# TuringLang/AdvancedHMC.jl

Measured on AMD Instinct MI355X. Metric: leapfrog-steps/sec (whole node) at n_chains x D, higher is better.
Workload: dtype f64

## Files before the change

advancedhmc.jl_amd/csrc/ahmc_device.hpp:

```cpp
#pragma once

#include <hip/hip_runtime.h>
#include <stdint.h>

namespace ahmc {

enum : uint32_t { RNG_MOMENTUM = 0, RNG_TRANSITION = 1, RNG_JITTER = 2, RNG_FINDEPS = 3 };
constexpr uint32_t COUPLED_CHAIN = 0xFFFFFFFFu;

struct Philox4 {
  uint32_t v[4];
};

__device__ __forceinline__ Philox4 philox4x32_10(uint32_t c0, uint32_t c1, uint32_t c2, uint32_t c3,
                                                 uint32_t k0, uint32_t k1) {
  constexpr uint32_t M0 = 0xD2511F53u, M1 = 0xCD9E8D57u, W0 = 0x9E3779B9u, W1 = 0xBB67AE85u;
#pragma unroll
  for (int round = 0; round < 10; ++round) {
    uint32_t hi0 = __umulhi(M0, c0), lo0 = M0 * c0;
    uint32_t hi1 = __umulhi(M1, c2), lo1 = M1 * c2;
    uint32_t n0 = hi1 ^ c1 ^ k0, n2 = hi0 ^ c3 ^ k1;
    c0 = n0; c1 = lo1; c2 = n2; c3 = lo0;
    k0 += W0; k1 += W1;
  }
// ... 154 lines not shown
__device__ __forceinline__ float leaf_weight_exp(float x) { return exp(x); }

template <class T, bool UNIFORM>
__device__ __forceinline__ T alpha_from_logweight(T lw) {
  const T w = leaf_weight_exp<UNIFORM>(lw > T(0) ? T(0) : lw);
  return w >= T(1) ? T(1) : w;
}

template <int LA, int LB>
__device__ __forceinline__ double leaf_weight_exp_pair(double x, bool odd) {
  constexpr auto C = [](unsigned long long bits) { return __builtin_bit_cast(double, bits); };
  const double xc = x < -1100.0 ? -1100.0 : x;
  const double dk = __builtin_rint(xc * 92.33248261689366);
  double t = __builtin_fma(dk, -0x1.62e42fef00000p-7, xc);
  t = __builtin_fma(dk, -0x1.473de6af278edp-40, t);
  const int k = (int)dk;
  const int ka = __builtin_amdgcn_readlane(k, LA), kb = __builtin_amdgcn_readlane(k, LB);
  const double tja = C(EXP2_64_BITS[ka & 63]), tjb = C(EXP2_64_BITS[kb & 63]);
  const double tj = odd ? tjb : tja;
  double q = __builtin_fma(t, 8.3333333333333332e-03, 4.1666666666666664e-02);
  q = fma3(t, q, 1.6666666666666666e-01);
  q = fma3(t, q, 0.5);
  q = fma3(t, q, 1.0);
  q = q * t;
  return __builtin_ldexp(__builtin_fma(tj, q, tj), k >> 6);
}
template <int LA, int LB>
__device__ __forceinline__ float leaf_weight_exp_pair(float x, bool) { return exp(x); }

template <int L0>
__device__ __forceinline__ double leaf_weight_exp_quad(double x, bool odd, bool up) {
  constexpr auto C = [](unsigned long long bits) { return __builtin_bit_cast(double, bits); };
  const double xc = x < -1100.0 ? -1100.0 : x;
  const double dk = __builtin_rint(xc * 92.33248261689366);
  double t = __builtin_fma(dk, -0x1.62e42fef00000p-7, xc);
  t = __builtin_fma(dk, -0x1.473de6af278edp-40, t);
  const int k = (int)dk;
  const int k0 = __builtin_amdgcn_readlane(k, L0), k1 = __builtin_amdgcn_readlane(k, L0 + 1);
  const int k2 = __builtin_amdgcn_readlane(k, L0 + 2), k3 = __builtin_amdgcn_readlane(k, L0 + 3);
  const double tj0 = C(EXP2_64_BITS[k0 & 63]), tj1 = C(EXP2_64_BITS[k1 & 63]);
  const double tj2 = C(EXP2_64_BITS[k2 & 63]), tj3 = C(EXP2_64_BITS[k3 & 63]);
  const double tjl = odd ? tj1 : tj0, tjh = odd ? tj3 : tj2;
  const double tj = up ? tjh : tjl;
  double q = __builtin_fma(t, 8.3333333333333332e-03, 4.1666666666666664e-02);
  q = fma3(t, q, 1.6666666666666666e-01);
  q = fma3(t, q, 0.5);
  q = fma3(t, q, 1.0);
  q = q * t;
  return __builtin_ldexp(__builtin_fma(tj, q, tj), k >> 6);
}
template <int L0>
__device__ __forceinline__ float leaf_weight_exp_quad(float x, bool, bool) { return exp(x); }

template <class T> __device__ __forceinline__ T maxabs(T a, T b) { return fabs(a) > fabs(b) ? a : b; }

template <int CTRL> __device__ __forceinline__ int dpp_i32(int v) {
  return __builtin_amdgcn_mov_dpp(v, CTRL, 0xf, 0xf, true);
}
template <int CTRL> __device__ __forceinline__ float dpp_mov(float v) {
  return __int_as_float(dpp_i32<CTRL>(__float_as_int(v)));
}
template <int CTRL> __device__ __forceinline__ double dpp_mov(double v) {
  int lo = __double2loint(v), hi = __double2hiint(v);
  return __hiloint2double(dpp_i32<CTRL>(hi), dpp_i32<CTRL>(lo));
}
__device__ __forceinline__ float swz16(float v) {
  return __int_as_float(__builtin_amdgcn_ds_swizzle(__float_as_int(v), 0x401F));
}
__device__ __forceinline__ double swz16(double v) {
  int lo = __builtin_amdgcn_ds_swizzle(__double2loint(v), 0x401F);
  int hi = __builtin_amdgcn_ds_swizzle(__double2hiint(v), 0x401F);
  return __hiloint2double(hi, lo);
}
__device__ __forceinline__ float xor16_sum(float v) {
  auto p = __builtin_amdgcn_permlane16_swap(__float_as_int(v), __float_as_int(v), false, false);
  return __int_as_float(p[0]) + __int_as_float(p[1]);
}
__device__ __forceinline__ double xor16_sum(double v) {
  auto lo = __builtin_amdgcn_permlane16_swap(__double2loint(v), __double2loint(v), false, false);
  auto hi = __builtin_amdgcn_permlane16_swap(__double2hiint(v), __double2hiint(v), false, false);
  return __hiloint2double(hi[0], lo[0]) + __hiloint2double(hi[1], lo[1]);
}
__device__ __forceinline__ float xor32_sum(float v) {
  auto p = __builtin_amdgcn_permlane32_swap(__float_as_int(v), __float_as_int(v), false, false);
  return __int_as_float(p[0]) + __int_as_float(p[1]);
}
__device__ __forceinline__ double xor32_sum(double v) {
  auto lo = __builtin_amdgcn_permlane32_swap(__double2loint(v), __double2loint(v), false, false);
  auto hi = __builtin_amdgcn_permlane32_swap(__double2hiint(v), __double2hiint(v), false, false);
  return __hiloint2double(hi[0], lo[0]) + __hiloint2double(hi[1], lo[1]);
}

#ifndef AHMC_MFMA_REDUCE
#define AHMC_MFMA_REDUCE 0
#endif
template <class T> struct MfmaRed;
template <> struct MfmaRed<double> {
  typedef double acc_t __attribute__((ext_vector_type(4)));
  static __device__ __forceinline__ acc_t mma(double a, double b, acc_t c) { return __builtin_amdgcn_mfma_f64_16x16x4f64(a, b, c, 0, 0, 0); }
  static constexpr unsigned SEL = 8u;
  static constexpr int RA = 0, RB = 2;
};
template <> struct MfmaRed<float> {
  typedef float acc_t __attribute__((ext_vector_type(4)));
  static __device__ __forceinline__ acc_t mma(float a, float b, acc_t c) { return __builtin_amdgcn_mfma_f32_16x16x4f32(a, b, c, 0, 0, 0); }
  static constexpr unsigned SEL = 1u;
// ... 107 lines not shown

#ifndef AHMC_PAIR_RED_QUAD
#define AHMC_PAIR_RED_QUAD 1
#endif
template <class T, int Q = AHMC_PAIR_RED_QUAD>
__device__ __forceinline__ bool wave64_pair_reduce(T da, T db, T& ea, T& eb) {
  static_assert(Q >= 0 && Q <= 3, "a row has four quads");
  const bool odd = (threadIdx.x & 1u) != 0, up = (threadIdx.x & 2u) != 0;
  const T x = (odd ? db : da) + dpp_mov<0xB1>(odd ? da : db);
  const T y = (odd ? eb : ea) + dpp_mov<0xB1>(odd ? ea : eb);
  T z = (up ? y : x) + dpp_mov<0x4E>(up ? x : y);
  z += dpp_mov<0x124>(z);
  z += dpp_mov<0x128>(z);
  z = xor16_sum(z);
  z = xor32_sum(z);
  const bool le0 = (__builtin_amdgcn_ballot_w64(z <= T(0)) & 3ull) != 0ull;
  ea = dpp_mov<0x150 + 4 * Q + 2>(z);
  eb = dpp_mov<0x150 + 4 * Q + 3>(z);
  return le0;
}
template <class T>
__device__ __forceinline__ bool wave64_pair_reduce_t(T da, T db, T ea, T eb, T& z) {
  const bool odd = (threadIdx.x & 1u) != 0, up = (threadIdx.x & 2u) != 0;
  const T x = (odd ? db : da) + dpp_mov<0xB1>(odd ? da : db);
  const T y = (odd ? eb : ea) + dpp_mov<0xB1>(odd ? ea : eb);
  z = (up ? y : x) + dpp_mov<0x4E>(up ? x : y);
  z += dpp_mov<0x124>(z);
  z += dpp_mov<0x128>(z);
  z = xor16_sum(z);
  z = xor32_sum(z);
  return (__builtin_amdgcn_ballot_w64(z <= T(0)) & 3ull) != 0ull;
}

template <class T>
__device__ __forceinline__ T wave64_quad_pair(T a, T b) {
  const bool odd = (threadIdx.x & 1u) != 0;
  return (odd ? b : a) + dpp_mov<0xB1>(odd ? a : b);
}
template <class T>
__device__ __forceinline__ unsigned long long wave64_quad_reduce_t(T xab, T xcd, T xl, T yab, T ycd, T& w) {
  const bool up = (threadIdx.x & 2u) != 0, oq = (threadIdx.x & 4u) != 0, hq = (threadIdx.x & 8u) != 0;
  const T rd = (up ? xcd : xab) + dpp_mov<0x4E>(up ? xab : xcd);
  const T re = (up ? ycd : yab) + dpp_mov<0x4E>(up ? yab : ycd);
  const T rl = xl + dpp_mov<0x4E>(xl);
  const T z = (oq ? re : rd) + dpp_mov<0x124>(oq ? rd : re);
  const T zl = rl + dpp_mov<0x124>(rl);
  w = (hq ? zl : z) + dpp_mov<0x128>(hq ? z : zl);
  w = xor16_sum(w);
  w = xor32_sum(w);
  return __builtin_amdgcn_ballot_w64(w <= T(0));
}
constexpr unsigned long long QUAD_TURN_AB = 0x3ull, QUAD_TURN_CD = 0xCull, QUAD_TURN_L1 = 0x300ull;

template <int G, class T, int K>
__device__ __forceinline__ void wave_allsum(T (&v)[K]) {
  static_assert(G == 1 || G == 2 || G == 4 || G == 8 || G == 16 || G == 32 || G == 64, "bad group size");
  if constexpr (G >= 16 && K == 4) {
    wave_allsum4<G>(v[0], v[1], v[2], v[3]);
    return;
  }
  if constexpr (G >= 16 && K % 2 == 0) {
#pragma unroll
    for (int k = 0; k < K; k += 2) wave_allsum2<G>(v[k], v[k + 1]);
    return;
  }
  if constexpr (G >= 2) {
#pragma unroll
    for (int k = 0; k < K; ++k) v[k] += dpp_mov<0xB1>(v[k]);
  }
  if constexpr (G >= 4) {
#pragma unroll
    for (int k = 0; k < K; ++k) v[k] += dpp_mov<0x4E>(v[k]);
  }
  if constexpr (G >= 8) {
#pragma unroll
    for (int k = 0; k < K; ++k) v[k] += dpp_mov<0x141>(v[k]);
  }
  if constexpr (G >= 16) {
#pragma unroll
    for (int k = 0; k < K; ++k) v[k] += dpp_mov<0x140>(v[k]);
  }
  if constexpr (G >= 32) {
#pragma unroll
    for (int k = 0; k < K; ++k) {
      if constexpr ((AHMC_DS_REDUCE & 1) != 0) v[k] += ds_swz<SWZ_XOR16>(v[k]); else v[k] = xor16_sum(v[k]);
    }
  }
  if constexpr (G >= 64) {
#pragma unroll
    for (int k = 0; k < K; ++k) {
      if constexpr ((AHMC_DS_REDUCE & 1) != 0) v[k] += ds_xor32(v[k]); else v[k] = xor32_sum(v[k]);
    }
  }
}
__device__ __forceinline__ double* xwave_buf() {
  __shared__ __attribute__((aligned(16))) double buf[8 * 8];
  return buf;
}

template <int G, class T, int K>
__device__ __forceinline__ void group_allsum(T (&v)[K]) {
  if constexpr (G <= 64) {
    wave_allsum<G>(v);
  } else {
    static_assert(G == 128 || G == 256 || G == 512, "bad multi-wave group size");
    static_assert(K <= 8, "at most 8 values per reduction");
// ... 365 lines not shown
  }
  const unsigned long long m_redo = __builtin_amdgcn_ballot_w64(lw > lw_limit);
  const unsigned long long m_div = __builtin_amdgcn_ballot_w64(!(-H0 < delta_max + ne));
  o.w[0] = readlane_t<LA>(w);
  o.w[1] = readlane_t<LB>(w);
  o.sa[0] = readlane_t<LA>(sa);
  o.sa[1] = readlane_t<LB>(sa);
  o.dH[0] = readlane_t<LA>(dH);
  o.dH[1] = readlane_t<LB>(dH);
  o.redo[0] = LINW && ((m_redo >> LA) & 1ull) != 0ull;
  o.redo[1] = LINW && ((m_redo >> LB) & 1ull) != 0ull;
  o.div[0] = ((m_div >> LA) & 1ull) != 0ull;
  o.div[1] = ((m_div >> LB) & 1ull) != 0ull;
}

__device__ __forceinline__ float readlane_at(float v, int l) { return __int_as_float(__builtin_amdgcn_readlane(__float_as_int(v), l)); }
__device__ __forceinline__ double readlane_at(double v, int l) {
  return __hiloint2double(__builtin_amdgcn_readlane(__double2hiint(v), l), __builtin_amdgcn_readlane(__double2loint(v), l));
}
template <class T> struct QuadLeafStats {
  static constexpr int L0 = 4;
  T w_l, sa_l, dH_l;
  unsigned long long m_redo, m_div;
  __device__ __forceinline__ T w(int k) const { return readlane_at(w_l, L0 + k); }
  __device__ __forceinline__ T sa(int k) const { return readlane_at(sa_l, L0 + k); }
  __device__ __forceinline__ T dH(int k) const { return readlane_at(dH_l, L0 + k); }
  __device__ __forceinline__ bool redo(int k) const { return ((m_redo >> (L0 + k)) & 1ull) != 0ull; }
  __device__ __forceinline__ bool div(int k) const { return ((m_div >> (L0 + k)) & 1ull) != 0ull; }
};
template <class T, bool LINW>
__device__ __forceinline__ void quad_leaf_stats(T wz, T H0, T delta_max, T lw_limit, QuadLeafStats<T>& o) {
  constexpr int L0 = QuadLeafStats<T>::L0;
  const bool odd = (threadIdx.x & 1u) != 0, up = (threadIdx.x & 2u) != 0, oq = (threadIdx.x & 4u) != 0;
  const T from_prev = dpp_mov<0x124>(wz);
  const T ne = neg_energy_sanitized(oq ? wz : from_prev);
  const T dH = -ne - H0;
  const T lw = H0 + ne;
  T w, sa;
  if constexpr (LINW) {
    w = leaf_weight_exp_quad<L0>(lw, odd, up);
    sa = w >= T(1) ? T(1) : w;
  } else {
    const T wa = leaf_weight_exp_quad<L0>(lw > T(0) ? T(0) : lw, odd, up);
    sa = wa >= T(1) ? T(1) : wa;
    w = lw;
  }
  o.m_redo = LINW ? __builtin_amdgcn_ballot_w64(lw > lw_limit) : 0ull;
  o.m_div = __builtin_amdgcn_ballot_w64(!(-H0 < delta_max + ne));
  o.w_l = w;
  o.sa_l = sa;
  o.dH_l = dH;
}

template <class T, int G, int E, int TK, class F>
__device__ __forceinline__ void leapfrog_step_plus2(Point<T, E>& z, const T (&minv)[E], T eps, const TargetP<T>& tp, int lane, int d0,
                                                    T (&extra)[2], F&& partials, bool use_pre = false) {
  const T eh = eps / 2;
#pragma unroll
  for (int e = 0; e < E; ++e) z.r[e] = leapfrog_kick(z.r[e], eh, z.g[e]);
#pragma unroll
  for (int e = 0; e < E; ++e) z.th[e] = leapfrog_drift(z.th[e], eps, minv[e], z.r[e]);
  T red[4];
  red[0] = target_eval<T, G, E, TK>(tp, z.th, z.g, lane, d0, use_pre);
#pragma unroll
  for (int e = 0; e < E; ++e) z.r[e] = leapfrog_kick(z.r[e], eh, z.g[e]);
  red[1] = kinetic_partial(z.r, minv);
  partials(red[2], red[3]);
  hier_publish_next<T, G, E, TK>(z, minv, eps);
  leapfrog_allsum<G, TK>(red);
  z.lp = sanitize(red[0]);
  z.lk = sanitize(-red[1] / 2);
  extra[0] = red[2];
  extra[1] = red[3];
}

template <class T, int G, int E, int TK>
__device__ __forceinline__ void fill_caches(Point<T, E>& z, const T (&minv)[E], const TargetP<T>& tp, int lane, int d0) {
  T red[2];
  red[0] = target_eval<T, G, E, TK>(tp, z.th, z.g, lane, d0);
  red[1] = kinetic_partial(z.r, minv);
  leapfrog_allsum<G, TK>(red);
  z.lp = sanitize(red[0]);
  z.lk = sanitize(-red[1] / 2);
}

template <class T, int E, bool SB = false>
__device__ __forceinline__ void load_vec(T (&v)[E], const T* __restrict__ base, int64_t off, int d0, int D, T pad) {
  constexpr int CH = (E * sizeof(T) >= 16) ? (int)(16 / sizeof(T)) : E;
  if constexpr (SB) {
    const T* sb = base + off;
    if (CH > 1 && d0 + E <= D && (reinterpret_cast<uintptr_t>(sb) % (CH * sizeof(T)) == 0)) {
      using V = T __attribute__((ext_vector_type(CH)));
      unsigned bv = (unsigned)d0 * (unsigned)sizeof(T);
      asm("; full lane" : "+v"(bv));
      const T* ptr = reinterpret_cast<const T*>(reinterpret_cast<const char*>(sb) + bv);
#pragma unroll
      for (int e = 0; e < E; e += CH) {
        V t = *reinterpret_cast<const V*>(ptr + e);
#pragma unroll
        for (int k = 0; k < CH; ++k) v[e + k] = t[k];
      }
    } else {
#pragma unroll
      for (int e = 0; e < E; ++e) {
        v[e] = pad;
        if (d0 + e < D) {
// ... 69 lines not shown
```

advancedhmc.jl_amd/csrc/ahmc_nuts.hpp:

```cpp
#pragma once

#ifndef AHMC_LEAF_PROF
#define AHMC_LEAF_PROF 0
#endif
#if AHMC_LEAF_PROF
#undef AHMC_WAVE_TIMELINE
#define AHMC_WAVE_TIMELINE 1
#define AHMC_TL_WORDS 24
#define AHMC_LP_TICK(i) { __builtin_amdgcn_sched_barrier(0); const unsigned n_ = (unsigned)__builtin_amdgcn_readfirstlane((int)(unsigned)__builtin_readcyclecounter()); __builtin_amdgcn_sched_barrier(0); lp_t[i] += n_ - lp_c; lp_c = n_; }
#define AHMC_LP_COUNT(i, n) { lp_t[i] += (unsigned)(n); }
#else
#define AHMC_LP_TICK(i)
#define AHMC_LP_COUNT(i, n)
#endif
#ifndef AHMC_WAVE_TIMELINE
#define AHMC_WAVE_TIMELINE 0
#endif
#ifndef AHMC_TL_WORDS
#define AHMC_TL_WORDS 8
#endif

#include <type_traits>

#include "ahmc_kernels.hpp"
// ... 129 lines not shown

template <class T, int G, int E, int TK, bool TEMPER = true>
__device__ __forceinline__ void leapfrog_core(Point<T, E>& z, const T (&minv)[E], T eps, const TargetP<T>& tp,
                                              const LeapfrogP<T>& lf, int lane, int d0) {
  if constexpr (TEMPER) temper(lf, z.r, 1, true, 1);
  const T eh = eps / 2;
#pragma unroll
  for (int e = 0; e < E; ++e) z.r[e] = leapfrog_kick(z.r[e], eh, z.g[e]);
#pragma unroll
  for (int e = 0; e < E; ++e) z.th[e] = leapfrog_drift(z.th[e], eps, minv[e], z.r[e]);
  (void)target_eval<T, G, E, TK>(tp, z.th, z.g, lane, d0);
#pragma unroll
  for (int e = 0; e < E; ++e) z.r[e] = leapfrog_kick(z.r[e], eh, z.g[e]);
  if constexpr (TEMPER) temper(lf, z.r, 1, false, 1);
}

template <bool WIDE>
struct DrawStreamT {
  static constexpr uint32_t PERIOD = !WIDE ? 4u : 256u;
  Rng rng;
  uint32_t k;
  Philox4 blk;
  __device__ __forceinline__ uint32_t lane_block() const {
    if constexpr (!WIDE) return 0u;
    else return threadIdx.x & 63u;
  }
  __device__ __forceinline__ void init(const Rng& r) { rng = r; k = 0; }
  __device__ __forceinline__ void resume(const Rng& r, uint32_t k0) {
    rng = r;
    k = k0;
    if (k & (PERIOD - 1u)) blk = rng.raw(RNG_TRANSITION, ((k & ~(PERIOD - 1u)) >> 2) + lane_block());
  }
  __device__ __forceinline__ uint32_t word() {
    if ((k & (PERIOD - 1u)) == 0u) blk = rng.raw(RNG_TRANSITION, (k >> 2) + lane_block());
    const uint32_t lo = (k & 1u) ? blk.v[1] : blk.v[0], hi = (k & 1u) ? blk.v[3] : blk.v[2];
    uint32_t w = (k & 2u) ? hi : lo;
    if constexpr (WIDE) {
      const uint32_t ks = (uint32_t)__builtin_amdgcn_readfirstlane((int)k);
      const int src = (int)((ks >> 2) & 63u);
      w = (uint32_t)__builtin_amdgcn_readlane((int)w, src);
    }
    ++k;
    return w;
  }
  __device__ __forceinline__ double uniform() { return ((double)word() + 0.5) * 2.3283064365386962890625e-10; }
  __device__ __forceinline__ bool boolean() { return (word() >> 31) != 0; }
  __device__ __forceinline__ double randexp() { return -log(uniform()); }
};
typedef DrawStreamT<false> DrawStream;

template <class T, int E, int MODE>
constexpr bool nuts_quad_step() { return true; }

template <class T, int G, int E, int MODE, int TK>
__global__ __launch_bounds__((G > 256 ? G : 256), (E >= 16 ? 1 : (MODE == 2 ? (E <= 2 ? 3 : 2) : (E <= 2 ? 4 : (E <= 4 ? 3 : 2))))) void k_nuts(KP<T> p) {
  constexpr int CPW = G >= 64 ? 1 : 64 / G;
  if constexpr (G == 64 && (MODE == 0 || MODE == 3)) {
    const unsigned int wave_id = blockIdx.x * (blockDim.x >> 6) + (threadIdx.x >> 6);
    if (wave_id >= p.n_chunks) {
      const unsigned int tw = (unsigned int)__builtin_amdgcn_readfirstlane((int)(wave_id - p.n_chunks));
      const int64_t rows = (int64_t)p.tail_n_trans * p.N, row0 = (int64_t)tw * p.tail_rows;
      if (tw < p.tail_waves && row0 < rows)
        normals_rows(p, p.tail_out, p.tail_iteration, (uint32_t)RNG_MOMENTUM, row0, row0 + p.tail_rows < rows ? row0 + p.tail_rows : rows, (int)(threadIdx.x & 63));
      return;
    }
  }
#define AHMC_UNI(b) (CPW == 1 ? (__builtin_amdgcn_ballot_w64(b) != 0) : (b))
#define AHMC_ANY(b) (CPW == 1 ? (bool)(b) : (__builtin_amdgcn_ballot_w64(b) != 0))
  constexpr int NCH = Chunking<T, E>::NCH, CH = Chunking<T, E>::CH;
  constexpr int SLOT_ELEMS = NCH * 64 * CH;
  extern __shared__ __attribute__((aligned(16))) unsigned char smem[];
  const int nwaves = blockDim.x >> 6;
  const int wib = threadIdx.x >> 6;
  const int lane64 = threadIdx.x & 63;
  int lane = (int)(threadIdx.x & (G - 1));
  int gi = G >= 64 ? 0 : lane64 / G;
  int d0 = lane * E;
  const int NLEV = p.max_depth > 1 ? p.max_depth - 1 : 1;
  constexpr bool LINW = MODE == 0 || MODE == 3;
  constexpr bool GENERAL = MODE == 2;
  constexpr bool FUSE_M0 = !GENERAL && G > 64;
  constexpr bool ADAPT = MODE >= 3;
  constexpr bool UTURN_ANY = G == 64;
  constexpr bool PAIR = G == 64 && !GENERAL && UTURN_ANY && !AHMC_MFMA_REDUCE && (AHMC_DS_REDUCE & 3) == 0 &&
                        !AHMC_LEAF_PROF && !AHMC_WAVE_TIMELINE;
  constexpr bool QUAD = PAIR && nuts_quad_step<T, E, MODE>();
  const bool strict = GENERAL && p.criterion == 2;
  const int NV = strict ? 3 : 2;
  const int n_slots = NV * NLEV + NUTS_DORMANT + NUTS_CKPT;
  const int CK0 = NV * NLEV + NUTS_DORMANT;
  const int n_lds_slots = p.n_lds_levels;
  T* lds_vec = reinterpret_cast<T*>(smem) + (size_t)wib * n_lds_slots * SLOT_ELEMS;
  T* sT = reinterpret_cast<T*>(smem) + (size_t)nwaves * n_lds_slots * SLOT_ELEMS + (size_t)wib * NUTS_NSC * NLEV * CPW;
  T* sAT = reinterpret_cast<T*>(smem) + (size_t)nwaves * (n_lds_slots * SLOT_ELEMS + NUTS_NSC * NLEV * CPW) + (size_t)wib * NUTS_NAT * CPW;
  int* sIbase = reinterpret_cast<int*>(reinterpret_cast<T*>(smem) + (size_t)nwaves * (n_lds_slots * SLOT_ELEMS + (NUTS_NSC * NLEV + NUTS_NAT) * CPW));
  int* sI = sIbase + (size_t)wib * NUTS_NSI * NLEV * CPW;
  int* sAI = sIbase + (size_t)nwaves * NUTS_NSI * NLEV * CPW + (size_t)wib * NUTS_NAI * CPW;
#define A_EPSNOM sAT[0 * CPW + gi]
#define A_DAEPS sAT[1 * CPW + gi]
#define A_DAMU sAT[2 * CPW + gi]
#define A_DAXBAR sAT[3 * CPW + gi]
#define A_DAHBAR sAT[4 * CPW + gi]
#define A_DAM sAI[0 * CPW + gi]
#define A_WVN sAI[1 * CPW + gi]
#define A_CHK sAI[2 * CPW + gi]
#define S_W(lvl) sT[((0) * NLEV + (lvl)) * CPW + gi]
#define S_CK(lvl) sI[((1) * NLEV + (lvl)) * CPW + gi]
  constexpr bool TSC = G == 64 && !GENERAL;
  const int64_t wave_slot = (int64_t)blockIdx.x * nwaves + wib;
  Slots<T, E, QUAD> sl;
  sl.lds = (AHMC_AS_LDS T*)lds_vec;
  if constexpr (QUAD) sl.glb = (AHMC_AS_GLB T*)(p.scratch + wave_scalar64(wave_slot) * (int64_t)(n_slots - n_lds_slots) * SLOT_ELEMS);
  else sl.glb = (AHMC_AS_GLB T*)(p.scratch + wave_slot * (int64_t)(n_slots - n_lds_slots) * SLOT_ELEMS);
  sl.n_lds = n_lds_slots;
  sl.lane_off = (unsigned)lane64 * CH;
  const int DORM = NV * NLEV;
  const int NL_HOT = NLEV < 4 ? NLEV : 4;
  const int HOT_END = 2 * NL_HOT - 1;
  const int COLD_DORM = HOT_END + 2 + 2 * (NLEV > 4 ? NLEV - 4 : 0);
  auto LA = [&](int l) -> int {
    if constexpr (GENERAL) return NV * l;
    else return l == 0 ? 0 : (l < NL_HOT ? 2 * l - 1 : HOT_END + 2 + 2 * (l - 4));
  };
  auto LRF = [&](int l) -> int {
    if constexpr (GENERAL) return NV * l + 1;
    else return l == 0 ? 0 : (l < NL_HOT ? 2 * l : HOT_END + 3 + 2 * (l - 4));
  };
  auto DS = [&](int k) -> int {
    if constexpr (GENERAL) return DORM + k;
    else return k == SL_TREE_A ? HOT_END : (k == SL_OTH_R ? HOT_END + 1
                : COLD_DORM + (k == SL_OTH_TH ? 0 : k == SL_OTH_G ? 1 : k == SL_Z0_R ? 2 : k == SL_Z0_G ? 3 : 4));
  };
  const bool classic = GENERAL && p.criterion == 0;
  const bool slice = GENERAL && p.sampler == 2;

  const unsigned int chunk = G > 64 ? blockIdx.x : blockIdx.x * nwaves + wib;
  if (chunk >= p.n_chunks) return;
  const int64_t slot = (int64_t)chunk * CPW + gi;
  const int64_t c = slot < p.N ? (p.order ? (int64_t)p.order[slot] : slot) : p.N;
// ... 105 lines not shown
      const int v = vleft ? -1 : 1;
      const bool need_swap = AHMC_UNI(!done && (vleft != cur_is_left));
      if (AHMC_ANY(need_swap)) {
        if (need_swap) {
          if (jw > 0) {
            Point<T, E> t;
            sl.load(DS(SL_OTH_TH), t.th);
            sl.load(DS(SL_OTH_R), t.r);
            sl.load(DS(SL_OTH_G), t.g);
            sl.store(DS(SL_OTH_TH), cur.th);
            sl.store(DS(SL_OTH_R), cur.r);
            sl.store(DS(SL_OTH_G), cur.g);
            copy_vec(cur.th, t.th);
            copy_vec(cur.r, t.r);
            copy_vec(cur.g, t.g);
          }
          int ti = pos_cur; pos_cur = pos_oth; pos_oth = ti;
          cur_is_left = vleft;
        }
      }
      if (strict && AHMC_ANY(!done)) {
        if (!done) sl.store(DS(SL_START_R), cur.r);
      }
      if (CKPT && jw >= CKPT_MIN_JW) {
        bool ck_save = true;
        if constexpr (CPW == 1) ck_save = AHMC_UNI(!done && pos_cur != 0);
        if (ck_save) {
          const unsigned xo = (unsigned)(((A_CHK & 1) ^ 1) * 3 * SLOT_ELEMS);
          sl.store_cold(CK0 + 0, xo, cur.th);
          sl.store_cold(CK0 + 1, xo, cur.r);
          sl.store_cold(CK0 + 2, xo, cur.g);
        }
      }
      const uint32_t nleaf = 1u << jw;
      bool alive = !done;
      bool sub_term = false;
      T A_c[E], RF_c[E];
      T w_c = 0, sa_c = 0, dh_c = 0;
      int na_c = 0, ck_c = 0;
      AHMC_LP_TICK(5)
      for (uint32_t leaf = 1; leaf <= nleaf; ++leaf) {
        if (!AHMC_ANY(alive)) break;
        AHMC_LP_COUNT(8, 1)
#if AHMC_WAVE_TIMELINE
        tl_steps += 1;
        tl_alive += (unsigned long long)__builtin_popcountll(__builtin_amdgcn_ballot_w64(alive && lane == 0));
#endif
        bool pair = false;
        if constexpr (PAIR) {
          pair = jw > 0;
          if (pair) ++leaf;
          if constexpr (QUAD) {
            if (jw > 1) leaf += 2;
          }
        }
        const int nm = __builtin_ctz(leaf);
        T dots_m0[2] = {0, 0}, RF_m0[E];
        if (pair) {
          if constexpr (PAIR) {
            if (QUAD && jw > 1) {
              const T es = v > 0 ? eps : -eps;
              T dab[2] = {0, 0}, dcd[2] = {0, 0}, dl[2] = {0, 0};
              const T e_a = leapfrog_step_ne_partial<T, G, E, TK>(cur, minv, es, p.tp, lane, d0);
              copy_vec(RF_c, cur.r);
              const T e_b = leapfrog_step_ne_partial<T, G, E, TK>(cur, minv, es, p.tp, lane, d0);
#pragma unroll
              for (int e = 0; e < E; ++e) {
                A_c[e] = RF_c[e] + cur.r[e];
                dab[0] += A_c[e] * (minv[e] * RF_c[e]);
                dab[1] += A_c[e] * (minv[e] * cur.r[e]);
              }
              const T yab = wave64_quad_pair(e_a, e_b), xab = wave64_quad_pair(dab[0], dab[1]);
              const T e_c = leapfrog_step_ne_partial<T, G, E, TK>(cur, minv, es, p.tp, lane, d0);
              T r_c[E];
              copy_vec(r_c, cur.r);
              const T e_d = leapfrog_step_ne_partial<T, G, E, TK>(cur, minv, es, p.tp, lane, d0);
#pragma unroll
              for (int e = 0; e < E; ++e) {
                const T rho_cd = r_c[e] + cur.r[e];
                dcd[0] += rho_cd * (minv[e] * r_c[e]);
                dcd[1] += rho_cd * (minv[e] * cur.r[e]);
                A_c[e] = A_c[e] + rho_cd;
                dl[0] += A_c[e] * (minv[e] * RF_c[e]);
                dl[1] += A_c[e] * (minv[e] * cur.r[e]);
              }
              T w_t;
              const unsigned long long turns =
                  wave64_quad_reduce_t(xab, wave64_quad_pair(dcd[0], dcd[1]), wave64_quad_pair(dl[0], dl[1]), yab, wave64_quad_pair(e_c, e_d), w_t);
              QuadLeafStats<T> qs;
              quad_leaf_stats<T, LINW>(w_t, H0, p.delta_max, sizeof(T) == 4 ? T(60) : T(LINW_LIMIT), qs);
              auto leaf_apply = [&](const int i) {
                pos_cur += v;
                ck_c = pos_cur;
                w_c = qs.w(i);
                if constexpr (LINW) redo = redo || qs.redo(i);
                sub_term = qs.div(i);
                numerical = numerical || sub_term;
                sa_c = sa_c + qs.sa(i);
                na_c = na_c + 1;
                const T dH_i = qs.dH(i);
                if (v > 0) { dh_c = maxabs(dh_c, dH_i); asm volatile(""); }
                else { dh_c = maxabs(dH_i, dh_c); asm volatile(""); }
              };
              auto merge_apply = [&](const T w_p, const int ck_p, const bool turn) {
                T w_new;
                if constexpr (LINW) w_new = w_p + w_c; else w_new = logaddexp(w_p, w_c);
                bool keep_first;
                if constexpr (LINW) keep_first = AHMC_UNI((T)ds.uniform() * w_new < w_p); else keep_first = AHMC_UNI(w_new < w_p + (T)ds.randexp());
                if (keep_first) ck_c = ck_p;
                w_c = w_new;
                sub_term = turn;
                AHMC_LP_COUNT(9, 1)
              };
              auto pair_apply = [&](const int h, const bool turn) {
                leaf_apply(2 * h);
                if (!sub_term) {
                  const T w_p = w_c;
                  const int ck_p = ck_c;
                  leaf_apply(2 * h + 1);
                  if (!sub_term) merge_apply(w_p, ck_p, turn);
                }
              };
              pair_apply(0, (turns & QUAD_TURN_AB) != 0ull);
              if (!sub_term) {
                const T w_ab = w_c;
                const int ck_ab = ck_c;
                pair_apply(1, (turns & QUAD_TURN_CD) != 0ull);
                if (!sub_term) merge_apply(w_ab, ck_ab, (turns & QUAD_TURN_L1) != 0ull);
              }
            } else {
              const T es = v > 0 ? eps : -eps;
              T ea = leapfrog_step_ne_partial<T, G, E, TK>(cur, minv, es, p.tp, lane, d0);
              T r_a[E];
              copy_vec(r_a, cur.r);
              T eb = leapfrog_step_ne_partial<T, G, E, TK>(cur, minv, es, p.tp, lane, d0);
              T dots[2] = {0, 0};
#pragma unroll
              for (int e = 0; e < E; ++e) {
                A_c[e] = r_a[e] + cur.r[e];
                dots[0] += A_c[e] * (minv[e] * r_a[e]);
                dots[1] += A_c[e] * (minv[e] * cur.r[e]);
              }
              T z_t;
              const bool turn_ab = wave64_pair_reduce_t(dots[0], dots[1], ea, eb, z_t);
              PairLeafStats<T> ps;
              pair_leaf_stats<T, LINW>(z_t, H0, p.delta_max, sizeof(T) == 4 ? T(60) : T(LINW_LIMIT), ps);
              auto leaf_apply = [&](const int i) {
                pos_cur += v;
                ck_c = pos_cur;
                w_c = ps.w[i];
                if constexpr (LINW) redo = redo || ps.redo[i];
                sub_term = ps.div[i];
                numerical = numerical || sub_term;
                sa_c = sa_c + ps.sa[i];
                na_c = na_c + 1;
                if (v > 0) { dh_c = maxabs(dh_c, ps.dH[i]); asm volatile(""); }
                else { dh_c = maxabs(ps.dH[i], dh_c); asm volatile(""); }
              };
              leaf_apply(0);
              if (!sub_term) {
                const T w_p = w_c;
                const int ck_p = ck_c;
                leaf_apply(1);
                if (!sub_term) {
                  T w_new;
                  if constexpr (LINW) w_new = w_p + w_c; else w_new = logaddexp(w_p, w_c);
                  bool keep_first;
                  if constexpr (LINW) keep_first = AHMC_UNI((T)ds.uniform() * w_new < w_p); else keep_first = AHMC_UNI(w_new < w_p + (T)ds.randexp());
                  if (keep_first) ck_c = ck_p;
                  w_c = w_new;
                  sub_term = turn_ab;
                  copy_vec(RF_c, r_a);
                  AHMC_LP_COUNT(9, 1)
                }
              }
            }
          }
        } else if (alive) {
          T ne_leaf = 0;
          if constexpr (GENERAL) {
            leapfrog_step<T, G, E, TK, true>(cur, minv, v > 0 ? eps : -eps, p.tp, p.lf, lane, d0, 1, 1);
          } else if (FUSE_M0 && nm > 0) {
// ... 106 lines not shown
                A_c[e] = A_p[e];
              }
              group_allsum<G>(dots);
              sub_term = (dots[0] >= 0) || (dots[1] >= 0);
            } else if (!strict) {
              T dots[2] = {dots_m0[0], dots_m0[1]};
              if constexpr (!pre.value) {
                dots[0] = 0;
                dots[1] = 0;
#pragma unroll
                for (int e = 0; e < E; ++e) {
                  A_c[e] = A_p[e] + A_in[e];
                  dots[0] += A_c[e] * (minv[e] * RF_p[e]);
                  dots[1] += A_c[e] * (minv[e] * cur.r[e]);
                }
                if constexpr (!UTURN_ANY) group_allsum<G>(dots);
              }
              if constexpr (UTURN_ANY && !pre.value) sub_term = wave64_any_le0_pair(dots[0], dots[1]);
              else sub_term = AHMC_UNI(dots[0] <= 0) || AHMC_UNI(dots[1] <= 0);
            } else {
              T RL_p[E];
              sl.load(NV * lvl + 2, RL_p);
              T dots[6] = {0, 0, 0, 0, 0, 0};
#pragma unroll
              for (int e = 0; e < E; ++e) {
                const T rho = A_p[e] + A_in[e];
                const T rho2 = A_p[e] + RF_in[e];
                const T rho3 = RL_p[e] + A_in[e];
                dots[0] += rho * (minv[e] * RF_p[e]);
                dots[1] += rho * (minv[e] * cur.r[e]);
                dots[2] += rho2 * (minv[e] * RF_p[e]);
                dots[3] += rho2 * (minv[e] * RF_in[e]);
                dots[4] += rho3 * (minv[e] * RL_p[e]);
                dots[5] += rho3 * (minv[e] * cur.r[e]);
                A_c[e] = rho;
              }
              group_allsum<G>(dots);
              sub_term = (dots[0] <= 0) || (dots[1] <= 0) || (dots[2] <= 0) || (dots[3] <= 0) || (dots[4] <= 0) || (dots[5] <= 0);
            }
            if constexpr (pre.value) copy_vec(RF_c, RF_m0); else copy_vec(RF_c, RF_p);
            AHMC_LP_COUNT(9, 1)
          }
        };
        if constexpr (GENERAL) {
          for (int lvl = 0; lvl < nm; ++lvl) {
            const bool m = AHMC_UNI(alive && !sub_term);
            if (!AHMC_ANY(m)) break;
            if (m) merge_level(lvl, A_c, RF_c, std::false_type{});
          }
        } else if (nm > 0) {
          bool m = AHMC_UNI(alive && !sub_term);
          if (AHMC_ANY(m)) {
            if (m && !pair) merge_level(0, cur.r, cur.r, std::bool_constant<FUSE_M0>{});
            for (int lvl = 1 + (QUAD && jw > 1 ? 1 : 0); lvl < nm; ++lvl) {
              m = AHMC_UNI(alive && !sub_term);
              if (!AHMC_ANY(m)) break;
              if (m) merge_level(lvl, A_c, RF_c, std::false_type{});
            }
          }
        }
        AHMC_LP_TICK(3)
        if (alive && sub_term) {
          alive = false;
        } else if (alive && leaf < nleaf) {
          if (GENERAL || nm > 0) {
            sl.store(LA(nm), A_c);
            sl.store(LRF(nm), RF_c);
          } else {
            sl.store(LA(0), cur.r);
          }
          if (strict) sl.store(NV * nm + 2, cur.r);
          S_W(nm) = w_c;
          S_CK(nm) = ck_c;
        }
        AHMC_LP_TICK(4)
      }
      if constexpr (!GENERAL) {
        if (jw == 0) {
          copy_vec(A_c, cur.r);
          copy_vec(RF_c, cur.r);
        }
      }
      if (!done) {
        if (!sub_term) {
          ++depth;
          bool acc;
          if (slice) acc = w_tree * (T)ds.uniform() < w_c;
          else if constexpr (LINW) acc = AHMC_UNI((T)ds.uniform() * w_tree < w_c);
          else acc = AHMC_UNI(w_tree < w_c + (T)ds.randexp());
          if (acc) {
            ck_tree = ck_c;
            if constexpr (CKPT) {
              const int start = pos_cur - v * (int)nleaf;
              int chk = A_CHK;
              if (jw >= CKPT_MIN_JW && start != 0) chk = (start << 1) | ((chk & 1) ^ 1);
              else if (((chk >> 1) > 0) != (v > 0) || (chk >> 1) == 0) chk = chk & 1;
              A_CHK = chk;
            }
          }
        }
        sa_tree = sa_tree + sa_c;
        na_tree = na_tree + na_c;
        dh_tree = v < 0 ? maxabs(dh_c, dh_tree) : maxabs(dh_tree, dh_c);
        if constexpr (LINW) w_tree = w_tree + w_c; else w_tree = slice ? w_tree + w_c : logaddexp(w_tree, w_c);
        bool turn;
        T oth_r[E];
        sl.load(DS(SL_OTH_R), oth_r);
        if (classic) {
          T oth_th[E];
          sl.load(DS(SL_OTH_TH), oth_th);
// ... 235 lines not shown
```

Before: 4.128 billion.

## Batch eight NUTS leapfrog leaves per doubling step with octet wave reductions

Extends the quad-leaf NUTS path to an eight-leaf (octet) path for small E, f64 non-MODE-1, TK==0 configurations when the tree depth allows. Two quad leapfrog blocks are computed back to back, and their U-turn dot products and energies are reduced in one combined DPP/permlane16_swap wave reduction with one batched exp for leaf weights. Merge levels are then applied from ballot masks. The aim is to amortise cross-lane reductions and per-level merge overhead across more leaves. In exchange it adds register pressure, an LDS spill/reload of A/RF, and wasted leapfrog work when a subtree terminates early within the eight.

```diff
diff --git a/advancedhmc.jl_amd/csrc/ahmc_device.hpp b/advancedhmc.jl_amd/csrc/ahmc_device.hpp
--- a/advancedhmc.jl_amd/csrc/ahmc_device.hpp
+++ b/advancedhmc.jl_amd/csrc/ahmc_device.hpp
@@ -230,6 +230,41 @@
 template <int L0>
 __device__ __forceinline__ float leaf_weight_exp_quad(float x, bool, bool) { return exp(x); }
 
+__device__ __forceinline__ double sel_odd_rows(double a, double b) {
+  const int lo = __builtin_amdgcn_update_dpp(__double2loint(a), __double2loint(b), 0xE4, 0xA, 0xF, false);
+  const int hi = __builtin_amdgcn_update_dpp(__double2hiint(a), __double2hiint(b), 0xE4, 0xA, 0xF, false);
+  return __hiloint2double(hi, lo);
+}
+template <int L0, int L1>
+__device__ __forceinline__ double leaf_weight_exp_oct(double x, bool odd, bool up) {
+  constexpr auto C = [](unsigned long long bits) { return __builtin_bit_cast(double, bits); };
+  const double xc = x < -1100.0 ? -1100.0 : x;
+  const double dk = __builtin_rint(xc * 92.33248261689366);
+  double t = __builtin_fma(dk, -0x1.62e42fef00000p-7, xc);
+  t = __builtin_fma(dk, -0x1.473de6af278edp-40, t);
+  const int k = (int)dk;
+  const int k0 = __builtin_amdgcn_readlane(k, L0), k1 = __builtin_amdgcn_readlane(k, L0 + 1);
+  const int k2 = __builtin_amdgcn_readlane(k, L0 + 2), k3 = __builtin_amdgcn_readlane(k, L0 + 3);
+  const int k4 = __builtin_amdgcn_readlane(k, L1), k5 = __builtin_amdgcn_readlane(k, L1 + 1);
+  const int k6 = __builtin_amdgcn_readlane(k, L1 + 2), k7 = __builtin_amdgcn_readlane(k, L1 + 3);
+  const double tj0 = C(EXP2_64_BITS[k0 & 63]), tj1 = C(EXP2_64_BITS[k1 & 63]);
+  const double tj2 = C(EXP2_64_BITS[k2 & 63]), tj3 = C(EXP2_64_BITS[k3 & 63]);
+  const double tj4 = C(EXP2_64_BITS[k4 & 63]), tj5 = C(EXP2_64_BITS[k5 & 63]);
+  const double tj6 = C(EXP2_64_BITS[k6 & 63]), tj7 = C(EXP2_64_BITS[k7 & 63]);
+  const double tjl = odd ? tj1 : tj0, tjh = odd ? tj3 : tj2;
+  const double tjl2 = odd ? tj5 : tj4, tjh2 = odd ? tj7 : tj6;
+  const double tja = up ? tjh : tjl, tjb = up ? tjh2 : tjl2;
+  const double tj = sel_odd_rows(tja, tjb);
+  double q = __builtin_fma(t, 8.3333333333333332e-03, 4.1666666666666664e-02);
+  q = fma3(t, q, 1.6666666666666666e-01);
+  q = fma3(t, q, 0.5);
+  q = fma3(t, q, 1.0);
+  q = q * t;
+  return __builtin_ldexp(__builtin_fma(tj, q, tj), k >> 6);
+}
+template <int L0, int L1>
+__device__ __forceinline__ float leaf_weight_exp_oct(float x, bool, bool) { return exp(x); }
+
 template <class T> __device__ __forceinline__ T maxabs(T a, T b) { return fabs(a) > fabs(b) ? a : b; }
 
 template <int CTRL> __device__ __forceinline__ int dpp_i32(int v) {
@@ -443,6 +478,39 @@
 }
 constexpr unsigned long long QUAD_TURN_AB = 0x3ull, QUAD_TURN_CD = 0xCull, QUAD_TURN_L1 = 0x300ull;
 
+template <class T>
+__device__ __forceinline__ T wave64_oct_rows_de(T xab, T xcd, T yab, T ycd) {
+  const bool up = (threadIdx.x & 2u) != 0, oq = (threadIdx.x & 4u) != 0;
+  const T rd = (up ? xcd : xab) + dpp_mov<0x4E>(up ? xab : xcd);
+  const T re = (up ? ycd : yab) + dpp_mov<0x4E>(up ? yab : ycd);
+  return (oq ? re : rd) + dpp_mov<0x124>(oq ? rd : re);
+}
+template <class T>
+__device__ __forceinline__ T wave64_oct_rows(T z, T xl, T xl2) {
+  const bool up = (threadIdx.x & 2u) != 0, hq = (threadIdx.x & 8u) != 0;
+  const T rl = (up ? xl2 : xl) + dpp_mov<0x4E>(up ? xl : xl2);
+  const T zl = rl + dpp_mov<0x124>(rl);
+  return (hq ? zl : z) + dpp_mov<0x128>(hq ? z : zl);
+}
+__device__ __forceinline__ float xor16_sum_t(float h1, float h2) {
+  auto p = __builtin_amdgcn_permlane16_swap(__float_as_int(h1), __float_as_int(h2), false, false);
+  return __int_as_float(p[0]) + __int_as_float(p[1]);
+}
+__device__ __forceinline__ double xor16_sum_t(double h1, double h2) {
+  auto lo = __builtin_amdgcn_permlane16_swap(__double2loint(h1), __double2loint(h2), false, false);
+  auto hi = __builtin_amdgcn_permlane16_swap(__double2hiint(h1), __double2hiint(h2), false, false);
+  return __hiloint2double(hi[0], lo[0]) + __hiloint2double(hi[1], lo[1]);
+}
+template <class T>
+__device__ __forceinline__ unsigned long long wave64_oct_reduce_t(T h1, T h2, T& w) {
+  w = xor16_sum_t(h1, h2);
+  w = xor32_sum(w);
+  return __builtin_amdgcn_ballot_w64(w <= T(0));
+}
+constexpr unsigned long long OCT_TURN_AB = QUAD_TURN_AB, OCT_TURN_CD = QUAD_TURN_CD, OCT_TURN_ABCD = QUAD_TURN_L1;
+constexpr unsigned long long OCT_TURN_EF = QUAD_TURN_AB << 16, OCT_TURN_GH = QUAD_TURN_CD << 16, OCT_TURN_EFGH = QUAD_TURN_L1 << 16;
+constexpr unsigned long long OCT_TURN_L2 = 0xC00ull << 16;
+
 template <int G, class T, int K>
 __device__ __forceinline__ void wave_allsum(T (&v)[K]) {
   static_assert(G == 1 || G == 2 || G == 4 || G == 8 || G == 16 || G == 32 || G == 64, "bad group size");
@@ -914,6 +982,43 @@
   o.dH_l = dH;
 }
 
+template <class T> struct OctLeafStats {
+  static constexpr int L0 = 4, L1 = 20;
+  T w_l, sa_l, dH_l;
+  unsigned m_flags;
+  static constexpr unsigned LANES = (0xFu << L0) | (0xFu << L1);
+  static __device__ __forceinline__ int lane_of(int k) { return k < 4 ? L0 + k : L1 + (k - 4); }
+  __device__ __forceinline__ T w(int k) const { return readlane_at(w_l, lane_of(k)); }
+  __device__ __forceinline__ T sa(int k) const { return readlane_at(sa_l, lane_of(k)); }
+  __device__ __forceinline__ T dH(int k) const { return readlane_at(dH_l, lane_of(k)); }
+  __device__ __forceinline__ bool redo(int k) const { return ((m_flags >> (lane_of(k) + 8)) & 1u) != 0u; }
+  __device__ __forceinline__ bool div(int k) const { return ((m_flags >> lane_of(k)) & 1u) != 0u; }
+};
+template <class T, bool LINW>
+__device__ __forceinline__ void oct_leaf_stats(T wz, T H0, T delta_max, T lw_limit, OctLeafStats<T>& o) {
+  constexpr int L0 = OctLeafStats<T>::L0, L1 = OctLeafStats<T>::L1;
+  const bool odd = (threadIdx.x & 1u) != 0, up = (threadIdx.x & 2u) != 0, oq = (threadIdx.x & 4u) != 0;
+  const T from_prev = dpp_mov<0x124>(wz);
+  const T ne = neg_energy_sanitized(oq ? wz : from_prev);
+  const T dH = -ne - H0;
+  const T lw = H0 + ne;
+  T w, sa;
+  if constexpr (LINW) {
+    w = leaf_weight_exp_oct<L0, L1>(lw, odd, up);
+    sa = w >= T(1) ? T(1) : w;
+  } else {
+    const T wa = leaf_weight_exp_oct<L0, L1>(lw > T(0) ? T(0) : lw, odd, up);
+    sa = wa >= T(1) ? T(1) : wa;
+    w = lw;
+  }
+  const unsigned m_redo = LINW ? (unsigned)__builtin_amdgcn_ballot_w64(lw > lw_limit) : 0u;
+  const unsigned m_div = (unsigned)__builtin_amdgcn_ballot_w64(!(-H0 < delta_max + ne));
+  o.m_flags = (m_div & OctLeafStats<T>::LANES) | ((m_redo & OctLeafStats<T>::LANES) << 8);
+  o.w_l = w;
+  o.sa_l = sa;
+  o.dH_l = dH;
+}
+
 template <class T, int G, int E, int TK, class F>
 __device__ __forceinline__ void leapfrog_step_plus2(Point<T, E>& z, const T (&minv)[E], T eps, const TargetP<T>& tp, int lane, int d0,
                                                     T (&extra)[2], F&& partials, bool use_pre = false) {
diff --git a/advancedhmc.jl_amd/csrc/ahmc_nuts.hpp b/advancedhmc.jl_amd/csrc/ahmc_nuts.hpp
--- a/advancedhmc.jl_amd/csrc/ahmc_nuts.hpp
+++ b/advancedhmc.jl_amd/csrc/ahmc_nuts.hpp
@@ -205,6 +205,17 @@
 template <class T, int E, int MODE>
 constexpr bool nuts_quad_step() { return true; }
 
+__device__ __forceinline__ bool nuts_oct_doubling(int jw) {
+  asm volatile("" : "+s"(jw));
+  return jw > 2;
+}
+template <class T, int E, int MODE>
+constexpr bool nuts_oct_step() {
+  if (E > 2) return false;
+  if (sizeof(T) == 8 && MODE == 1) return false;
+  return true;
+}
+
 template <class T, int G, int E, int MODE, int TK>
 __global__ __launch_bounds__((G > 256 ? G : 256), (E >= 16 ? 1 : (MODE == 2 ? (E <= 2 ? 3 : 2) : (E <= 2 ? 4 : (E <= 4 ? 3 : 2))))) void k_nuts(KP<T> p) {
   constexpr int CPW = G >= 64 ? 1 : 64 / G;
@@ -238,6 +249,7 @@
   constexpr bool PAIR = G == 64 && !GENERAL && UTURN_ANY && !AHMC_MFMA_REDUCE && (AHMC_DS_REDUCE & 3) == 0 &&
                         !AHMC_LEAF_PROF && !AHMC_WAVE_TIMELINE;
   constexpr bool QUAD = PAIR && nuts_quad_step<T, E, MODE>();
+  constexpr bool OCT = QUAD && TK == 0 && nuts_oct_step<T, E, MODE>();
   const bool strict = GENERAL && p.criterion == 2;
   const int NV = strict ? 3 : 2;
   const int n_slots = NV * NLEV + NUTS_DORMANT + NUTS_CKPT;
@@ -449,6 +461,9 @@
           if (pair) ++leaf;
           if constexpr (QUAD) {
             if (jw > 1) leaf += 2;
+            if constexpr (OCT) {
+              if (nuts_oct_doubling(jw)) leaf += 4;
+            }
           }
         }
         const int nm = __builtin_ctz(leaf);
@@ -456,6 +471,113 @@
         if (pair) {
           if constexpr (PAIR) {
             if (QUAD && jw > 1) {
+              if constexpr (OCT) {
+              const T es = v > 0 ? eps : -eps;
+              auto quad_vec = [&](T (&RF_q)[E], T (&A_q)[E], T& xab, T& xcd, T& xl, T& yab, T& ycd) {
+                T dab[2] = {0, 0}, dcd[2] = {0, 0}, dl[2] = {0, 0};
+                const T e_a = leapfrog_step_ne_partial<T, G, E, TK>(cur, minv, es, p.tp, lane, d0);
+                copy_vec(RF_q, cur.r);
+                const T e_b = leapfrog_step_ne_partial<T, G, E, TK>(cur, minv, es, p.tp, lane, d0);
+#pragma unroll
+                for (int e = 0; e < E; ++e) {
+                  A_q[e] = RF_q[e] + cur.r[e];
+                  dab[0] += A_q[e] * (minv[e] * RF_q[e]);
+                  dab[1] += A_q[e] * (minv[e] * cur.r[e]);
+                }
+                yab = wave64_quad_pair(e_a, e_b);
+                xab = wave64_quad_pair(dab[0], dab[1]);
+                const T e_c = leapfrog_step_ne_partial<T, G, E, TK>(cur, minv, es, p.tp, lane, d0);
+                T r_c[E];
+                copy_vec(r_c, cur.r);
+                const T e_d = leapfrog_step_ne_partial<T, G, E, TK>(cur, minv, es, p.tp, lane, d0);
+#pragma unroll
+                for (int e = 0; e < E; ++e) {
+                  const T rho_cd = r_c[e] + cur.r[e];
+                  dcd[0] += rho_cd * (minv[e] * r_c[e]);
+                  dcd[1] += rho_cd * (minv[e] * cur.r[e]);
+                  A_q[e] = A_q[e] + rho_cd;
+                  dl[0] += A_q[e] * (minv[e] * RF_q[e]);
+                  dl[1] += A_q[e] * (minv[e] * cur.r[e]);
+                }
+                xcd = wave64_quad_pair(dcd[0], dcd[1]);
+                xl = wave64_quad_pair(dl[0], dl[1]);
+                ycd = wave64_quad_pair(e_c, e_d);
+              };
+              auto leaf_apply = [&](const auto& st, const int i) {
+                pos_cur += v;
+                ck_c = pos_cur;
+                w_c = st.w(i);
+                if constexpr (LINW) redo = redo || st.redo(i);
+                sub_term = st.div(i);
+                numerical = numerical || sub_term;
+                sa_c = sa_c + st.sa(i);
+                na_c = na_c + 1;
+                const T dH_i = st.dH(i);
+                if (v > 0) { dh_c = maxabs(dh_c, dH_i); asm volatile(""); }
+                else { dh_c = maxabs(dH_i, dh_c); asm volatile(""); }
+              };
+              auto merge_apply = [&](const T w_p, const int ck_p, const bool turn) {
+                T w_new;
+                if constexpr (LINW) w_new = w_p + w_c; else w_new = logaddexp(w_p, w_c);
+                bool keep_first;
+                if constexpr (LINW) keep_first = AHMC_UNI((T)ds.uniform() * w_new < w_p); else keep_first = AHMC_UNI(w_new < w_p + (T)ds.randexp());
+                if (keep_first) ck_c = ck_p;
+                w_c = w_new;
+                sub_term = turn;
+                AHMC_LP_COUNT(9, 1)
+              };
+              auto pair_apply = [&](const auto& st, const int i0, const bool turn) {
+                leaf_apply(st, i0);
+                if (!sub_term) {
+                  const T w_p = w_c;
+                  const int ck_p = ck_c;
+                  leaf_apply(st, i0 + 1);
+                  if (!sub_term) merge_apply(w_p, ck_p, turn);
+                }
+              };
+              auto quad_apply = [&](const auto& st, const int i0, const bool turn_ab, const bool turn_cd, const bool turn_l1) {
+                pair_apply(st, i0, turn_ab);
+                if (!sub_term) {
+                  const T w_ab = w_c;
+                  const int ck_ab = ck_c;
+                  pair_apply(st, i0 + 2, turn_cd);
+                  if (!sub_term) merge_apply(w_ab, ck_ab, turn_l1);
+                }
+              };
+              T xab, xcd, xl, yab, ycd;
+              quad_vec(RF_c, A_c, xab, xcd, xl, yab, ycd);
+              const T h1 = wave64_oct_rows(wave64_oct_rows_de(xab, xcd, yab, ycd), xl, xl);
+              T h2 = h1;
+              if (nuts_oct_doubling(jw)) {
+                sl.store(LA(1), A_c);
+                sl.store(LRF(1), RF_c);
+                T RF_e[E], A_e[E];
+                quad_vec(RF_e, A_e, xab, xcd, xl, yab, ycd);
+                T z2 = wave64_oct_rows_de(xab, xcd, yab, ycd);
+                asm volatile("" : "+v"(z2));
+                sl.load(LA(1), A_c);
+                sl.load(LRF(1), RF_c);
+                T d2[2] = {0, 0};
+#pragma unroll
+                for (int e = 0; e < E; ++e) {
+                  A_c[e] = A_c[e] + A_e[e];
+                  d2[0] += A_c[e] * (minv[e] * RF_c[e]);
+                  d2[1] += A_c[e] * (minv[e] * cur.r[e]);
+                }
+                h2 = wave64_oct_rows(z2, xl, wave64_quad_pair(d2[0], d2[1]));
+              }
+              T w_t;
+              const unsigned turns = (unsigned)wave64_oct_reduce_t(h1, h2, w_t);
+              OctLeafStats<T> os;
+              oct_leaf_stats<T, LINW>(w_t, H0, p.delta_max, sizeof(T) == 4 ? T(60) : T(LINW_LIMIT), os);
+              quad_apply(os, 0, (turns & (unsigned)OCT_TURN_AB) != 0u, (turns & (unsigned)OCT_TURN_CD) != 0u, (turns & (unsigned)OCT_TURN_ABCD) != 0u);
+              if (!sub_term && nuts_oct_doubling(jw)) {
+                const T w_abcd = w_c;
+                const int ck_abcd = ck_c;
+                quad_apply(os, 4, (turns & (unsigned)OCT_TURN_EF) != 0u, (turns & (unsigned)OCT_TURN_GH) != 0u, (turns & (unsigned)OCT_TURN_EFGH) != 0u);
+                if (!sub_term) merge_apply(w_abcd, ck_abcd, (turns & (unsigned)OCT_TURN_L2) != 0u);
+              }
+              } else {
               const T es = v > 0 ? eps : -eps;
               T dab[2] = {0, 0}, dcd[2] = {0, 0}, dl[2] = {0, 0};
               const T e_a = leapfrog_step_ne_partial<T, G, E, TK>(cur, minv, es, p.tp, lane, d0);
@@ -525,6 +647,7 @@
                 pair_apply(1, (turns & QUAD_TURN_CD) != 0ull);
                 if (!sub_term) merge_apply(w_ab, ck_ab, (turns & QUAD_TURN_L1) != 0ull);
               }
+              }
             } else {
               const T es = v > 0 ? eps : -eps;
               T ea = leapfrog_step_ne_partial<T, G, E, TK>(cur, minv, es, p.tp, lane, d0);
@@ -737,10 +860,18 @@
           bool m = AHMC_UNI(alive && !sub_term);
           if (AHMC_ANY(m)) {
             if (m && !pair) merge_level(0, cur.r, cur.r, std::bool_constant<FUSE_M0>{});
+            if constexpr (OCT) {
+              for (int lvl = 1 + (jw > 1 ? 1 : 0) + (nuts_oct_doubling(jw) ? 1 : 0); lvl < nm; ++lvl) {
+                m = AHMC_UNI(alive && !sub_term);
+                if (!AHMC_ANY(m)) break;
+                if (m) merge_level(lvl, A_c, RF_c, std::false_type{});
+              }
+            } else {
             for (int lvl = 1 + (QUAD && jw > 1 ? 1 : 0); lvl < nm; ++lvl) {
               m = AHMC_UNI(alive && !sub_term);
               if (!AHMC_ANY(m)) break;
               if (m) merge_level(lvl, A_c, RF_c, std::false_type{});
+            }
             }
           }
         }
```

After: 4.432 billion (median of 6 runs). +7.4%, better.
